# facebookresearch/AVID-CMA

Measured on AMD Instinct MI355X. Metric: clips/sec (video+audio fwd+bwd+NCE+Adam), higher is better.
Workload: dtype f32 (bf16x3 MFMA)

## Files before the change

avid-cma_amd/csrc/common.h:

```cpp
#pragma once
#include <hip/hip_runtime.h>
#include <stdint.h>
#include <stdio.h>
#include <string.h>

#include <mutex>

#include "../../include/avid_hip.h"

namespace avid {

typedef float floatx4 __attribute__((ext_vector_type(4)));
typedef float floatx16 __attribute__((ext_vector_type(16)));

void set_error(const char* fmt, ...);

inline int check_launch(const char* what) {
  hipError_t e = hipGetLastError();
  if (e != hipSuccess) {
    set_error("%s: %s", what, hipGetErrorString(e));
    return AVID_E_HIP;
  }
  return AVID_OK;
}

#define AVID_REQUIRE(cond, code, ...) \
  do {                                \
    if (!(cond)) {                    \
      avid::set_error(__VA_ARGS__);   \
      return (code);                  \
    }                                 \
  } while (0)

int device_cus();

inline int64_t ceil_div(int64_t a, int64_t b) { return (a + b - 1) / b; }

struct ScopedTimer {
  hipStream_t s;
  int slot;
  ScopedTimer(hipStream_t stream, const char* name, double flops, double bytes);
  ~ScopedTimer();
};

struct Stage {
  void* host = nullptr;
  size_t bytes = 0;
  hipEvent_t done = nullptr;
  bool used = false;
};
extern std::mutex g_stage_mu;
Stage* take_stage(size_t bytes);

int sim_gemm_nt(const float* A, const float* Bq, float* C, const float* Cin, int op, long long M, int N, int K,
                hipStream_t s);

bool stem_fwd_supported(const avid_conv_desc* d);
bool stem_wgrad_supported(const avid_conv_desc* d);
size_t stem_fwd_ws_bytes(const avid_conv_desc* d);
size_t stem_wgrad_ws_bytes(const avid_conv_desc* d);
int stem_fwd(const avid_conv_desc* d, const float* x, const float* w, float* y, float* stats, void* ws, hipStream_t s);
int stem_fwd_grid(const avid_conv_desc* d);
bool stem_fwd_is_split(const avid_conv_desc* d);
bool stem_fwd_is_presplit(const avid_conv_desc* d);
int stem_wgrad(const avid_conv_desc* d, const float* x, const float* dy, float* dw, void* ws, hipStream_t s);

bool wino_supported(const avid_conv_desc* d, int mode);
int wino_variant(const avid_conv_desc* d, int mode);
size_t wino_ws_bytes(const avid_conv_desc* d, int mode);
int wino_grid(const avid_conv_desc* d, int mode);
// ... 160 lines not shown
```

avid-cma_amd/csrc/common.hip:

```cpp
#include <stdarg.h>
#include <stdlib.h>

#include <map>
#include <string>
#include <vector>

#include <atomic>
#include "common.h"

namespace avid {
static thread_local char g_err[512] = "";

void set_error(const char* fmt, ...) {
  va_list ap;
  va_start(ap, fmt);
  vsnprintf(g_err, sizeof(g_err), fmt, ap);
  va_end(ap);
}

struct TimingRec {
  const char* name;
  double flops, bytes;
  hipEvent_t e0, e1;
};
static bool g_timing = false;
static std::vector<TimingRec> g_recs;
static std::vector<hipEvent_t> g_pool;

static hipEvent_t get_event() {
  if (!g_pool.empty()) {
    hipEvent_t e = g_pool.back();
    g_pool.pop_back();
    return e;
  }
  hipEvent_t e;
  (void)hipEventCreate(&e);
  return e;
}

ScopedTimer::ScopedTimer(hipStream_t stream, const char* name, double flops, double bytes) : s(stream), slot(-1) {
  if (!g_timing) return;
  TimingRec r{name, flops, bytes, get_event(), get_event()};
  (void)hipEventRecord(r.e0, s);
  slot = (int)g_recs.size();
  g_recs.push_back(r);
}
ScopedTimer::~ScopedTimer() {
  if (slot >= 0) (void)hipEventRecord(g_recs[slot].e1, s);
}

std::mutex g_stage_mu;
static std::vector<Stage> g_stages;

Stage* take_stage(size_t bytes) {
  for (auto& s : g_stages)
    if (s.bytes >= bytes && (!s.used || hipEventQuery(s.done) == hipSuccess)) return &s;
  Stage s;
  s.bytes = bytes < (1u << 20) ? (1u << 20) : bytes * 2;
  if (hipHostMalloc(&s.host, s.bytes, hipHostMallocDefault) != hipSuccess) return nullptr;
  if (hipEventCreateWithFlags(&s.done, hipEventDisableTiming) != hipSuccess) {
    (void)hipHostFree(s.host);
    return nullptr;
  }
  g_stages.push_back(s);
  return &g_stages.back();
}

static std::atomic<int> g_cu_budget{-1};

static int physical_cus() {
  static int cus[64] = {0};
// ... 93 lines not shown
```

avid-cma_amd/csrc/conv.hip:

```cpp
#include <math.h>
#include <stdlib.h>

#include <atomic>
#include <type_traits>

#include "common.h"

namespace avid {

typedef unsigned int uintx4 __attribute__((ext_vector_type(4)));

struct ConvArgs {
  const float* __restrict__ src;
  const float* __restrict__ wk;
  int w_row, w_nrec;
  const float* __restrict__ addend;
  const float* __restrict__ bias;
  float* __restrict__ dst;
  float* __restrict__ part;
  int B, Ts, Hs, Ws, Cs;
  int Td, Hd, Wd, Cd;
  int kt, kh, kw;
  int st, sh, sw;
  int pt, ph, pw;
  int M;
  int mode;
  int relu;
  int epi_op;
  int nsplit, ksteps_per_split;
  int mt2_begin, mt2_count;
  int part_row_begin;
  long long ssB, ssT, ssH, ssW, ssC;
  int ncls, cls_ptiles_total;
  int cls_begin[9];
  int cls_p0[8][3], cls_n[8][3];
  int cls_d0[8][3], cls_nd[8][3];
  unsigned mgW, mgH, mgT;
// ... 2437 lines not shown
  }
  reinterpret_cast<floatx4*>(dw)[i] = s;
}

__global__ __launch_bounds__(256) void dx_scatter_strided_kernel(const float* __restrict__ compact, const float* __restrict__ addend,
                                                                 float* __restrict__ dx, long long n4, int c4, int Ti, int Hi, int Wi,
                                                                 int To, int Ho, int Wo, int st, int sh, int sw) {
  for (long long i = (long long)blockIdx.x * 256 + threadIdx.x; i < n4; i += (long long)gridDim.x * 256) {
    const int c = (int)(i % c4);
    long long r = i / c4;
    const int w = (int)(r % Wi); r /= Wi;
    const int h = (int)(r % Hi); r /= Hi;
    const int t = (int)(r % Ti);
    const long long b = r / Ti;
    floatx4 v = {0.f, 0.f, 0.f, 0.f};
    if (t % st == 0 && h % sh == 0 && w % sw == 0)
      v = reinterpret_cast<const floatx4*>(compact)[((((b * To + t / st) * Ho + h / sh) * Wo + w / sw)) * c4 + c];
    if (addend) v += reinterpret_cast<const floatx4*>(addend)[i];
    reinterpret_cast<floatx4*>(dx)[i] = v;
  }
}

__global__ void weight_transpose_kernel(const float* __restrict__ w, float* __restrict__ wt, int Co, int ntaps, int Ci) {
  long long i = (long long)blockIdx.x * blockDim.x + threadIdx.x;
  long long n = (long long)Co * ntaps * Ci;
  if (i >= n) return;
  int co = (int)(i % Co);
  long long r = i / Co;
  int tap = (int)(r % ntaps);
  int ci = (int)(r / ntaps);
  wt[i] = w[((long long)co * ntaps + tap) * Ci + ci];
}

__device__ __forceinline__ void weight_transform_body(const avid_wt_desc& d, float (*tile)[33]) {
  if (d.mode >= 5) {
    const int N = d.mode == 5 ? d.Cout : d.Cin, C = d.mode == 5 ? d.Cin : d.Cout;
    const int c8 = C / 8, cpt = C / 32, ntn = N / 64;
    const long long items = (long long)N * d.ntaps * c8;
    char* out = reinterpret_cast<char*>(d.wt);
    for (long long i = (long long)blockIdx.x * 256 + threadIdx.x; i < items; i += (long long)gridDim.x * 256) {
      int n, tap, k8;
      float v[8];
      if (d.mode == 5) {
        k8 = (int)(i % c8);
        const long long r = i / c8;
        tap = (int)(r % d.ntaps);
        n = (int)(r / d.ntaps);
        const floatx4* src = reinterpret_cast<const floatx4*>(d.w + ((long long)n * d.ntaps + tap) * C + k8 * 8);
        const floatx4 a = src[0], b = src[1];
        v[0] = a[0]; v[1] = a[1]; v[2] = a[2]; v[3] = a[3]; v[4] = b[0]; v[5] = b[1]; v[6] = b[2]; v[7] = b[3];
      } else {
        n = (int)(i % N);
        const long long r = i / N;
        k8 = (int)(r % c8);
        tap = (int)(r / c8);
#pragma unroll
        for (int e = 0; e < 8; ++e) v[e] = d.w[((long long)(k8 * 8 + e) * d.ntaps + tap) * d.Cin + n];
      }
      pk_bf16x8 fh, fm, fl;
      pk_split8(floatx4{v[0], v[1], v[2], v[3]}, floatx4{v[4], v[5], v[6], v[7]}, fh, fm, fl);
      const int cb = k8 >> 2, st = (k8 >> 1) & 1, hh = k8 & 1;
      const long long chunk = ((long long)tap * cpt + cb) * ntn + (n >> 6);
      char* o = out + chunk * PK_BCH + ((((n >> 5) & 1) * 2 + st) * 3) * 1024 + (hh * 32 + (n & 31)) * 16;
      *reinterpret_cast<pk_bf16x8*>(o) = fh;
      *reinterpret_cast<pk_bf16x8*>(o + 1024) = fm;
      *reinterpret_cast<pk_bf16x8*>(o + 2048) = fl;
    }
    return;
  }
  if (d.mode != 0) {
    const bool fwd = d.mode & 1;
    wino_weight_elements(d.w, d.wt, fwd ? d.Cout : d.Cin, fwd ? d.Cin : d.Cout, d.Cin, !fwd,
                         (long long)blockIdx.x * 256 + threadIdx.x, (long long)gridDim.x * 256, d.mode <= 2 ? 2 : (W2_SPLIT ? 3 : 1));
    return;
  }
  const int tco = (d.Cout + 31) / 32, tci = (d.Cin + 31) / 32;
  const long long ntile = (long long)tco * tci * d.ntaps;
  const int tx = threadIdx.x & 31, ty = threadIdx.x >> 5;
  for (long long t = blockIdx.x; t < ntile; t += gridDim.x) {
    const int ci0 = (int)(t % tci) * 32;
    const long long r = t / tci;
    const int co0 = (int)(r % tco) * 32;
    const int tap = (int)(r / tco);
#pragma unroll
    for (int k = 0; k < 4; ++k) {
      const int co = co0 + ty + 8 * k, ci = ci0 + tx;
      tile[ty + 8 * k][tx] = (co < d.Cout && ci < d.Cin) ? d.w[((long long)co * d.ntaps + tap) * d.Cin + ci] : 0.f;
    }
    __syncthreads();
#pragma unroll
    for (int k = 0; k < 4; ++k) {
      const int ci = ci0 + ty + 8 * k, co = co0 + tx;
      if (ci < d.Cin && co < d.Cout) d.wt[((long long)ci * d.ntaps + tap) * d.Cout + co] = tile[tx][ty + 8 * k];
    }
    __syncthreads();
  }
}

__global__ __launch_bounds__(256) void weight_transpose_batched_kernel(const avid_wt_desc* __restrict__ descs) {
  __shared__ float tile[32][33];
  const avid_wt_desc d = descs[blockIdx.y];
  weight_transform_body(d, tile);
}

__global__ __launch_bounds__(256) void weight_transform_kernel(const avid_wt_desc d) {
  __shared__ float tile[32][33];
  weight_transform_body(d, tile);
}

static int validate(const avid_conv_desc* d) {
  AVID_REQUIRE(d != nullptr, AVID_E_BADARG, "conv: null descriptor");
  AVID_REQUIRE(d->B > 0 && d->Ti > 0 && d->Hi > 0 && d->Wi > 0 && d->Cin > 0 && d->Cout > 0, AVID_E_SHAPE,
               "conv: non-positive dims");
  AVID_REQUIRE(d->kt > 0 && d->kh > 0 && d->kw > 0 && d->kt < 256 && d->kh < 256 && d->kw < 256, AVID_E_SHAPE,
               "conv: bad kernel extent");
  AVID_REQUIRE(d->st > 0 && d->sh > 0 && d->sw > 0, AVID_E_SHAPE, "conv: bad stride");
  const int To = (d->Ti + 2 * d->pt - d->kt) / d->st + 1;
  const int Ho = (d->Hi + 2 * d->ph - d->kh) / d->sh + 1;
  const int Wo = (d->Wi + 2 * d->pw - d->kw) / d->sw + 1;
  AVID_REQUIRE(To == d->To && Ho == d->Ho && Wo == d->Wo, AVID_E_SHAPE,
               "conv: output extent (%d,%d,%d) does not match (%d,%d,%d)", d->To, d->Ho, d->Wo, To, Ho, Wo);
  AVID_REQUIRE(d->Cout % 64 == 0, AVID_E_UNSUPPORTED, "conv: Cout=%d must be a multiple of 64", d->Cout);
  const bool vec = (d->Cin % 32 == 0) && !d->x_channel_first;
  const int ntaps = d->kt * d->kh * d->kw;
  if (!vec) {
    AVID_REQUIRE(ntaps * d->Cin <= KTAB_MAX - 32, AVID_E_UNSUPPORTED,
                 "conv: gather path supports K <= %d (got %d)", KTAB_MAX - 32, ntaps * d->Cin);
  } else {
    AVID_REQUIRE(d->kt <= 8 && d->kh <= 8 && d->kw <= 8, AVID_E_UNSUPPORTED, "conv: vector path supports kernel extents <= 8");
    AVID_REQUIRE((long long)d->Cout * ntaps * d->Cin * 4 < (1ll << 31), AVID_E_UNSUPPORTED, "conv: weights >= 2 GiB");
  }
  const long long M = (long long)d->B * d->To * d->Ho * d->Wo;
  const long long Mi = (long long)d->B * d->Ti * d->Hi * d->Wi;
  AVID_REQUIRE(M < (1ll << 31) && Mi < (1ll << 31), AVID_E_UNSUPPORTED, "conv: more than 2^31 pixels");
  const long long pix_in = (long long)d->Ti * d->Hi * d->Wi, pix_out = (long long)d->To * d->Ho * d->Wo;
  const long long span_in = (128 / pix_out + 2) * pix_in * d->Cin * 4;
  const long long span_out = (128 / pix_in + 2) * pix_out * d->Cout * 4;
  AVID_REQUIRE(span_in < (1ll << 31) && span_out < (1ll << 31), AVID_E_UNSUPPORTED,
               "conv: one batch item is too large for 32-bit tile offsets");
  return AVID_OK;
// ... 959 lines not shown

static bool dgrad_compactable(const avid_conv_desc* d) {
  return d->kt == 1 && d->kh == 1 && d->kw == 1 && (d->st > 1 || d->sh > 1 || d->sw > 1) && d->pt == 0 && d->ph == 0 &&
         d->pw == 0 && !d->x_channel_first && d->Cin % 4 == 0;
}
static avid_conv_desc dgrad_compact_desc(const avid_conv_desc* d) {
  avid_conv_desc c = *d;
  c.Ti = d->To; c.Hi = d->Ho; c.Wi = d->Wo;
  c.st = c.sh = c.sw = 1;
  return c;
}
static size_t dgrad_compact_bytes(const avid_conv_desc* d) {
  return (sizeof(float) * (size_t)d->B * d->To * d->Ho * d->Wo * d->Cin + 255) / 256 * 256;
}

extern "C" size_t avid_conv_dgrad_workspace_bytes(const avid_conv_desc* d) {
  if (!d || validate(d)) return 0;
  if (dgrad_compactable(d)) {
    const avid_conv_desc c = dgrad_compact_desc(d);
    return dgrad_compact_bytes(d) + avid_conv_dgrad_workspace_bytes(&c);
  }
  const long long M = (long long)d->B * d->Ti * d->Hi * d->Wi;
  const int nk = trim_taps(d).d.kt * d->kh * d->kw * (d->Cout / BK);
  size_t fl = igemm_ws_floats(M, d->Cin, nk, 1);
  if (d->st > 1 || d->sh > 1 || d->sw > 1) {
    const size_t want = (size_t)8 * (size_t)M * d->Cin;
    if (want > fl) fl = want;
  }
  size_t need = dgrad_wt_bytes(d) + sizeof(float) * fl;
  if (wino_supported(d, 1) && wino_ws_bytes(d, 1) > need) need = wino_ws_bytes(d, 1);
  return need;
}

extern "C" int avid_weight_transpose_batched(int n, const avid_wt_desc* descs_dev, int64_t max_elems,
                                             avid_stream_t stream) {
  AVID_REQUIRE(n > 0 && descs_dev && max_elems > 0, AVID_E_BADARG, "weight_transpose_batched: bad argument");
  hipStream_t s = (hipStream_t)stream;
  ScopedTimer t(s, "weight_transpose_batched_kernel", 0.0, 0.0);
  long long gx = ceil_div(max_elems, 1024);
  if (gx > 256) gx = 256;
  hipLaunchKernelGGL(weight_transpose_batched_kernel, dim3((unsigned)gx, (unsigned)n), dim3(256), 0, s, descs_dev);
  return check_launch("weight_transpose_batched");
}

extern "C" int avid_weight_transform(const avid_wt_desc* desc, avid_stream_t stream) {
  AVID_REQUIRE(desc && desc->w && desc->wt && desc->Cout > 0 && desc->Cin > 0 && desc->ntaps > 0 && desc->mode >= 0 && desc->mode <= 6,
               AVID_E_BADARG, "weight_transform: bad descriptor");
  AVID_REQUIRE(desc->mode < 5 || (desc->mode == 5 ? desc->Cout % 64 == 0 && desc->Cin % 32 == 0 : desc->Cin % 64 == 0 && desc->Cout % 32 == 0),
               AVID_E_UNSUPPORTED, "weight_transform: mode %d needs 64 | rows and 32 | channels", desc->mode);
  hipStream_t s = (hipStream_t)stream;
  ScopedTimer t(s, "weight_transform_kernel", 0.0, 0.0);
  long long gx = ceil_div((long long)desc->Cout * desc->ntaps * desc->Cin, 1024);
  if (gx > 256) gx = 256;
  hipLaunchKernelGGL(weight_transform_kernel, dim3((unsigned)gx), dim3(256), 0, s, *desc);
  return check_launch("weight_transform");
}

extern "C" int avid_conv_dgrad_bn_rows(const avid_conv_desc* d) {
  if (!d || validate(d)) return 0;
  if (d->x_channel_first || d->Cin % 64 || d->Cout % 32 || d->st > 2 || d->sh > 2 || d->sw > 2) return 0;
  if (wino_supported(d, 1)) return wino_grid(d, 1);
  if (d->Cin > 1024 || (256 % (d->Cin / 4)) != 0) return 0;
  const long long M = (long long)d->B * d->Ti * d->Hi * d->Wi;
  if (d->st > 1 || d->sh > 1 || d->sw > 1) {
    if (M * d->Cin * 4 >= (1ll << 31)) return 0;
    const Trim tr = trim_taps(d);
    ConvArgs a{};
    fill_common(a, &tr.d);
    a.Td = d->Ti; a.Hd = d->Hi; a.Wd = d->Wi; a.Cd = d->Cin;
    const int BN = d->Cin % 128 == 0 && s2_wide() ? 128 : 64;
    a.Cs = d->Cout;
    a.M = (int)M;
    const StridedPlan pl = plan_strided(a, 128, BN, (size_t)8 * (size_t)M * d->Cin);
    return pl.grid + (pl.any_split ? (int)ceil_div(M, stats_rpb(M, d->Cin)) : 0);
  }
  const PkPlan pk = plan_pk(M, d->Cin, trim_taps(d).d.kt * d->kh * d->kw * (d->Cout / BK), 1);
  return pk.grid + (pk.f > 1 ? (int)ceil_div(M - pk.tail_row0, stats_rpb(M - pk.tail_row0, d->Cin)) : 0);
}

extern "C" int avid_conv_dgrad(const avid_conv_desc* d, const float* dy, const float* w, const float* wt_in,
                               const float* u, const float* addend, const int32_t* addend_stride, float* dx, const avid_bn_bwd_fuse* bn,
                               void* ws, size_t ws_bytes, avid_stream_t stream) {
  int rc = validate(d);
  if (rc) return rc;
// ... 545 lines not shown
```

avid-cma_amd/csrc/norm_pool.hip:

```cpp
#include <math.h>
#include <stdlib.h>

#include "common.h"

namespace avid {

struct BnPlan {
  int G;
  int rows_per_pass;
  int rows_per_block;
  int nblk;
};

static BnPlan bn_plan(int64_t M, int C) {
  BnPlan p;
  p.G = C / 4;
  p.rows_per_pass = 256 / p.G;
  int64_t rpb = ceil_div(M, 1024);
  if (rpb < 16) rpb = 16;
  rpb = ceil_div(rpb, p.rows_per_pass) * p.rows_per_pass;
  p.rows_per_block = (int)rpb;
  p.nblk = (int)ceil_div(M, rpb);
  return p;
}
// ... 602 lines not shown
    const int g = (int)(i % G);
    long long r = i / G;
    const int w = (int)(r % W);
    r /= W;
    const int h = (int)(r % H);
    const long long bt = r / H;
    floatx4 acc = {0, 0, 0, 0};
#pragma unroll
    for (int dh = 0; dh < 3; ++dh) {
      const int nh = h + 1 - dh;
      if (nh < 0 || (nh & 1)) continue;
      const int ho = nh >> 1;
      if (ho >= Ho) continue;
#pragma unroll
      for (int dw = 0; dw < 3; ++dw) {
        const int nw = w + 1 - dw;
        if (nw < 0 || (nw & 1)) continue;
        const int wo = nw >> 1;
        if (wo >= Wo) continue;
        const long long o = ((bt * Ho + ho) * Wo + wo) * (long long)G + g;
        const uchar4 a = reinterpret_cast<const uchar4*>(am)[o];
        const floatx4 d = reinterpret_cast<const floatx4*>(dy)[o];
        const int slot = dh * 3 + dw;
        acc.x += a.x == slot ? d.x : 0.f;
        acc.y += a.y == slot ? d.y : 0.f;
        acc.z += a.z == slot ? d.z : 0.f;
        acc.w += a.w == slot ? d.w : 0.f;
      }
    }
    reinterpret_cast<floatx4*>(dx)[i] = acc;
  }
}

__global__ __launch_bounds__(256) void bn_pool_fwd_kernel(const float* __restrict__ x, const float* __restrict__ scale,
                                                          const float* __restrict__ shift, float* __restrict__ y,
                                                          uint8_t* __restrict__ am, int BT, int H, int W, int Ho, int Wo,
                                                          int G) {
  const long long n = (long long)BT * Ho * Wo * G;
  const long long stride = (long long)gridDim.x * blockDim.x;
  for (long long i = (long long)blockIdx.x * blockDim.x + threadIdx.x; i < n; i += stride) {
    const int g = (int)(i % G);
    long long r = i / G;
    const int wo = (int)(r % Wo);
    r /= Wo;
    const int ho = (int)(r % Ho);
    const long long bt = r / Ho;
    const floatx4 sc = reinterpret_cast<const floatx4*>(scale)[g];
    const floatx4 sh = reinterpret_cast<const floatx4*>(shift)[g];
    floatx4 best = {-INFINITY, -INFINITY, -INFINITY, -INFINITY};
    int slot[4] = {0, 0, 0, 0};
    bool first = true;
#pragma unroll
    for (int dh = 0; dh < 3; ++dh) {
      const int h = ho * 2 - 1 + dh;
      if ((unsigned)h >= (unsigned)H) continue;
#pragma unroll
      for (int dw = 0; dw < 3; ++dw) {
        const int w = wo * 2 - 1 + dw;
        if ((unsigned)w >= (unsigned)W) continue;
        const floatx4 xv = *reinterpret_cast<const floatx4*>(x + (((bt * H + h) * W + w) * (long long)G + g) * 4);
#pragma unroll
        for (int j = 0; j < 4; ++j) {
          const float v = fmaxf(fmaf(xv[j], sc[j], sh[j]), 0.f);
          if (first || v > best[j] || v != v) {
            best[j] = v;
            slot[j] = dh * 3 + dw;
          }
        }
        first = false;
      }
    }
    reinterpret_cast<floatx4*>(y)[i] = best;
    reinterpret_cast<uchar4*>(am)[i] = make_uchar4((unsigned char)slot[0], (unsigned char)slot[1],
                                                   (unsigned char)slot[2], (unsigned char)slot[3]);
  }
}

__global__ __launch_bounds__(256) void bn_pool_fwd_eval_kernel(const float* __restrict__ x, const float* __restrict__ scale,
                                                               const float* __restrict__ shift, float* __restrict__ y,
                                                               int BT, int H, int W, int Ho, int Wo, int G) {
  const long long n = (long long)BT * Ho * Wo * G;
  const long long stride = (long long)gridDim.x * blockDim.x;
  for (long long i = (long long)blockIdx.x * blockDim.x + threadIdx.x; i < n; i += stride) {
    const int g = (int)(i % G);
    long long r = i / G;
    const int wo = (int)(r % Wo);
    r /= Wo;
    const int ho = (int)(r % Ho);
    const long long bt = r / Ho;
    const floatx4 sc = reinterpret_cast<const floatx4*>(scale)[g];
    const floatx4 sh = reinterpret_cast<const floatx4*>(shift)[g];
    floatx4 best = {-INFINITY, -INFINITY, -INFINITY, -INFINITY};
    bool first = true;
#pragma unroll
    for (int dh = 0; dh < 3; ++dh) {
      const int h = ho * 2 - 1 + dh;
      if ((unsigned)h >= (unsigned)H) continue;
#pragma unroll
      for (int dw = 0; dw < 3; ++dw) {
        const int w = wo * 2 - 1 + dw;
        if ((unsigned)w >= (unsigned)W) continue;
        const floatx4 xv = *reinterpret_cast<const floatx4*>(x + (((bt * H + h) * W + w) * (long long)G + g) * 4);
#pragma unroll
        for (int j = 0; j < 4; ++j) {
          const float v = fmaxf(fmaf(xv[j], sc[j], sh[j]), 0.f);
          if (first || v > best[j] || v != v) best[j] = v;
        }
        first = false;
      }
    }
    reinterpret_cast<floatx4*>(y)[i] = best;
  }
}

struct PoolCell {
  floatx4 d[2][2];
};
__device__ __forceinline__ PoolCell pool_cell_grad(const float* __restrict__ dy, const uint8_t* __restrict__ am,
                                                   long long bt, int a, int b, int g, int Ho, int Wo, int G) {
  uchar4 A[2][2];
  floatx4 D[2][2];
#pragma unroll
  for (int i = 0; i < 2; ++i)
#pragma unroll
    for (int j = 0; j < 2; ++j) {
      const bool ok = a + i < Ho && b + j < Wo;
      const long long o = ((bt * Ho + (ok ? a + i : 0)) * Wo + (ok ? b + j : 0)) * (long long)G + g;
      A[i][j] = reinterpret_cast<const uchar4*>(am)[o];
      D[i][j] = reinterpret_cast<const floatx4*>(dy)[o];
      if (!ok) A[i][j] = make_uchar4(255, 255, 255, 255);
    }
  PoolCell c;
  auto pick = [](uchar4 s, int slot, floatx4 d) {
    floatx4 r;
    r.x = s.x == slot ? d.x : 0.f; r.y = s.y == slot ? d.y : 0.f;
    r.z = s.z == slot ? d.z : 0.f; r.w = s.w == slot ? d.w : 0.f;
    return r;
  };
  c.d[0][0] = pick(A[0][0], 1 * 3 + 1, D[0][0]);
  c.d[0][1] = pick(A[0][0], 1 * 3 + 2, D[0][0]) + pick(A[0][1], 1 * 3 + 0, D[0][1]);
  c.d[1][0] = pick(A[0][0], 2 * 3 + 1, D[0][0]) + pick(A[1][0], 0 * 3 + 1, D[1][0]);
  c.d[1][1] = pick(A[0][0], 2 * 3 + 2, D[0][0]) + pick(A[0][1], 2 * 3 + 0, D[0][1]) + pick(A[1][0], 0 * 3 + 2, D[1][0]) +
              pick(A[1][1], 0 * 3 + 0, D[1][1]);
  return c;
}
// ... 258 lines not shown
                     running_mean, running_var, eps, n4, C / 4, relu);
  return check_launch("bn_fwd_eval");
}

extern "C" int avid_bn_eval_coeffs_batched(int n, const avid_bn_eval_item* items_dev, avid_stream_t stream) {
  static_assert(sizeof(BnEvalItem) == sizeof(avid_bn_eval_item), "BnEvalItem mirrors avid_bn_eval_item");
  AVID_REQUIRE(n > 0 && n <= 65535, AVID_E_SHAPE, "bn_eval_coeffs_batched: n=%d outside [1, 65535]", n);
  AVID_REQUIRE(items_dev, AVID_E_BADARG, "bn_eval_coeffs_batched: null table");
  ScopedTimer t((hipStream_t)stream, "bn_eval_coeff_batched_kernel", 0.0, 32.0 * n * 256);
  hipLaunchKernelGGL(bn_eval_coeff_batched_kernel, dim3(4, (unsigned)n), dim3(256), 0, (hipStream_t)stream,
                     reinterpret_cast<const BnEvalItem*>(items_dev));
  return check_launch("bn_eval_coeffs_batched");
}

extern "C" int avid_bn_apply_eval(int64_t M, int C, const float* x, const float* scale, const float* shift, int relu, float* y,
                                  avid_stream_t stream) {
  int rc = bn_check(M, C, "bn_apply_eval");
  if (rc) return rc;
  AVID_REQUIRE(x && scale && shift && y, AVID_E_BADARG, "bn_apply_eval: null pointer");
  const long long n4 = (long long)M * (C / 4);
  ScopedTimer t((hipStream_t)stream, "bn_apply_kernel", 0.0, 8.0 * M * C);
  hipLaunchKernelGGL(bn_apply_kernel, dim3(ew_grid(n4)), dim3(256), 0, (hipStream_t)stream, x, y, scale, shift, n4, C / 4, relu);
  return check_launch("bn_apply_eval");
}

extern "C" int avid_bn_relu_maxpool_fwd_eval(int B, int T, int H, int W, int C, const float* x, const float* scale,
                                             const float* shift, float* y, avid_stream_t stream) {
  const int64_t M = (int64_t)B * T * H * W;
  int rc = bn_check(M, C, "bn_relu_maxpool_fwd_eval");
  if (rc) return rc;
  AVID_REQUIRE(B > 0 && T > 0 && H > 0 && W > 0, AVID_E_SHAPE, "bn_relu_maxpool_fwd_eval: bad shape");
  AVID_REQUIRE(x && scale && shift && y, AVID_E_BADARG, "bn_relu_maxpool_fwd_eval: null pointer");
  const int Ho = (H + 2 - 3) / 2 + 1, Wo = (W + 2 - 3) / 2 + 1;
  const long long n = (long long)B * T * Ho * Wo * (C / 4);
  ScopedTimer t((hipStream_t)stream, "bn_pool_fwd_eval_kernel", 0.0, 4.0 * B * T * C * ((double)H * W + Ho * Wo));
  hipLaunchKernelGGL(bn_pool_fwd_eval_kernel, dim3(ew_grid(n)), dim3(256), 0, (hipStream_t)stream, x, scale, shift, y, B * T, H,
                     W, Ho, Wo, C / 4);
  return check_launch("bn_relu_maxpool_fwd_eval");
}

extern "C" int avid_bn_bwd(int64_t M, int C, const float* x, const float* dy, const float* gamma,
                           const float* save_mean, const float* save_invstd, const float* save_scale,
                           const float* save_shift, int relu, float* dx, float* dgamma, float* dbeta,
                           const float* partials, int nparts, int frozen, void* ws, size_t ws_bytes,
                           avid_stream_t stream) {
  int rc = bn_check(M, C, "bn_bwd");
  if (rc) return rc;
  AVID_REQUIRE(x && dy && gamma && save_mean && save_invstd && dx && dgamma && dbeta && ws, AVID_E_BADARG,
               "bn_bwd: null pointer");
  AVID_REQUIRE(!relu || (save_scale && save_shift), AVID_E_BADARG, "bn_bwd: relu needs the saved scale/shift");
  AVID_REQUIRE(ws_bytes >= avid_bn_workspace_bytes(M, C), AVID_E_BADARG, "bn_bwd: workspace too small");
  hipStream_t s = (hipStream_t)stream;
  BnPlan p = bn_plan(M, C);
  float* wsf = static_cast<float*>(ws);
  float* k1 = wsf + (size_t)p.nblk * 2 * C;
  float* k2 = k1 + C;
  const float* part = wsf;
  int nblk = p.nblk;
  if (partials && nparts > 0) {
    part = partials;
    nblk = nparts;
  } else {
    ScopedTimer t(s, "bn_bwd_partial_kernel", 0.0, 4.0 * M * C * 2);
    hipLaunchKernelGGL(bn_bwd_partial_kernel, dim3(p.nblk), dim3(256), 0, s, x, save_scale, save_shift, dy, save_mean,
                       save_invstd, wsf,
                       (long long)M, C, p.G, p.rows_per_pass, p.rows_per_block, relu);
  }
  if (bn_fused_ok(M, C)) {
    ScopedTimer t(s, "bn_bwd_fin_apply_kernel", 0.0, 4.0 * M * C * 3);
    hipLaunchKernelGGL(bn_bwd_fin_apply_kernel, dim3(bn_fused_grid(M, C)), dim3(256), 0, s, part, nblk, (long long)M, C, x,
// ... 17 lines not shown

extern "C" int avid_bn_relu_maxpool_fwd(int B, int T, int H, int W, int C, const float* x, const float* gamma,
                                        const float* beta, float* running_mean, float* running_var, float momentum,
                                        float eps, float* y, uint8_t* argmax, float* save_mean, float* save_invstd,
                                        float* save_scale, float* save_shift, int64_t* num_batches_tracked,
                                        const float* partials, int nparts, void* ws, size_t ws_bytes,
                                        avid_stream_t stream) {
  const int64_t M = (int64_t)B * T * H * W;
  int rc = bn_check(M, C, "bn_relu_maxpool_fwd");
  if (rc) return rc;
  AVID_REQUIRE(B > 0 && T > 0 && H > 0 && W > 0, AVID_E_SHAPE, "bn_relu_maxpool_fwd: bad shape");
  AVID_REQUIRE(x && gamma && beta && y && argmax && save_mean && save_invstd && save_scale && save_shift && ws,
               AVID_E_BADARG, "bn_relu_maxpool_fwd: null pointer");
  AVID_REQUIRE(ws_bytes >= avid_bn_workspace_bytes(M, C), AVID_E_BADARG, "bn_relu_maxpool_fwd: workspace too small");
  hipStream_t s = (hipStream_t)stream;
  BnPlan p = bn_plan(M, C);
  const float* part = static_cast<float*>(ws);
  int nblk = p.nblk;
  if (partials && nparts > 0) {
    part = partials;
    nblk = nparts;
  } else {
    ScopedTimer t(s, "bn_stats_partial_kernel", 0.0, 4.0 * M * C);
    hipLaunchKernelGGL(bn_stats_partial_kernel, dim3(p.nblk), dim3(256), 0, s, x, static_cast<float*>(ws), (long long)M,
                       C, p.G, p.rows_per_pass, p.rows_per_block);
  }
  {
    ScopedTimer t(s, "bn_finalize_kernel", 0.0, 8.0 * nblk * C);
    hipLaunchKernelGGL(bn_finalize_kernel, dim3((unsigned)ceil_div(C, FIN_CH)), dim3(1024), 0, s, part, nblk,
                       (long long)M, C, gamma, beta, running_mean, running_var, momentum, eps, save_mean, save_invstd,
                       save_scale, save_shift, reinterpret_cast<long long*>(num_batches_tracked));
  }
  const int Ho = (H + 2 - 3) / 2 + 1, Wo = (W + 2 - 3) / 2 + 1;
  const long long n = (long long)B * T * Ho * Wo * p.G;
  {
    ScopedTimer t(s, "bn_pool_fwd_kernel", 0.0, 4.0 * B * T * C * ((double)H * W + 1.25 * Ho * Wo));
    hipLaunchKernelGGL(bn_pool_fwd_kernel, dim3(ew_grid(n)), dim3(256), 0, s, x, save_scale, save_shift, y, argmax, B * T,
                       H, W, Ho, Wo, p.G);
  }
  return check_launch("bn_relu_maxpool_fwd");
}

extern "C" int avid_bn_relu_maxpool_bwd(int B, int T, int H, int W, int C, const float* x, const float* dy,
                                        const uint8_t* argmax, const float* gamma, const float* save_mean,
                                        const float* save_invstd, const float* save_scale, const float* save_shift,
                                        float* dx, float* dgamma, float* dbeta, void* ws, size_t ws_bytes,
                                        avid_stream_t stream) {
  const int64_t M = (int64_t)B * T * H * W;
  int rc = bn_check(M, C, "bn_relu_maxpool_bwd");
  if (rc) return rc;
  AVID_REQUIRE(x && dy && argmax && gamma && save_mean && save_invstd && save_scale && save_shift && dx && dgamma &&
                   dbeta && ws,
               AVID_E_BADARG, "bn_relu_maxpool_bwd: null pointer");
  AVID_REQUIRE(ws_bytes >= avid_bn_workspace_bytes(M, C), AVID_E_BADARG, "bn_relu_maxpool_bwd: workspace too small");
  hipStream_t s = (hipStream_t)stream;
  BnPlan p = bn_plan(M, C);
  const int Ho = (H + 2 - 3) / 2 + 1, Wo = (W + 2 - 3) / 2 + 1;
  float* part = static_cast<float*>(ws);
  float* k1 = part + (size_t)p.nblk * 2 * C;
  float* k2 = k1 + C;
  const long long cells = (long long)B * T * ((H + 1) / 2) * ((W + 1) / 2);
  long long cpb = ceil_div(cells, p.nblk);
  cpb = ceil_div(cpb, p.rows_per_pass) * p.rows_per_pass;
  const int nblk = (int)ceil_div(cells, cpb);
  {
    ScopedTimer t(s, "bn_pool_bwd_partial_kernel", 0.0, 4.0 * M * C * 1.3);
    hipLaunchKernelGGL(bn_pool_bwd_partial_kernel, dim3(nblk), dim3(256), 0, s, x, save_scale, save_shift, dy, argmax,
                       save_mean, save_invstd, part, cells, C, p.G, p.rows_per_pass, (int)cpb, H, W, Ho, Wo);
  }
  {
    ScopedTimer t(s, "bn_bwd_finalize_kernel", 0.0, 8.0 * nblk * C);
// ... 75 lines not shown
```

Measured before the change: 7016.

## Stage packed weight transform through LDS and band bn-relu-maxpool rows

The packed-bf16 weight transform (modes 5/6) now processes one 64x32 chunk per block. It loads the weights with coalesced vector reads into LDS and writes the hi/mid/lo fragments contiguously, replacing the old scattered per-thread gathers. The fused BN+ReLU+maxpool forward now gives each thread a vertical band of output rows. Each thread reuses the overlapping input row between adjacent pooling windows and prefetches the next rows, which cuts redundant loads and activation work at the cost of fewer threads. Timing instrumentation also gains byte counts, read through a host sync only when timing is on.

```diff
diff --git a/avid-cma_amd/csrc/common.h b/avid-cma_amd/csrc/common.h
--- a/avid-cma_amd/csrc/common.h
+++ b/avid-cma_amd/csrc/common.h
@@ -36,6 +36,7 @@
 
 inline int64_t ceil_div(int64_t a, int64_t b) { return (a + b - 1) / b; }
 
+bool timing_on();
 struct ScopedTimer {
   hipStream_t s;
   int slot;
diff --git a/avid-cma_amd/csrc/common.hip b/avid-cma_amd/csrc/common.hip
--- a/avid-cma_amd/csrc/common.hip
+++ b/avid-cma_amd/csrc/common.hip
@@ -37,6 +37,8 @@
   (void)hipEventCreate(&e);
   return e;
 }
+
+bool timing_on() { return g_timing; }
 
 ScopedTimer::ScopedTimer(hipStream_t stream, const char* name, double flops, double bytes) : s(stream), slot(-1) {
   if (!g_timing) return;
diff --git a/avid-cma_amd/csrc/conv.hip b/avid-cma_amd/csrc/conv.hip
--- a/avid-cma_amd/csrc/conv.hip
+++ b/avid-cma_amd/csrc/conv.hip
@@ -3,6 +3,7 @@
 
 #include <atomic>
 #include <type_traits>
+#include <vector>
 
 #include "common.h"
 
@@ -2506,39 +2507,55 @@
   wt[i] = w[((long long)co * ntaps + tap) * Ci + ci];
 }
 
-__device__ __forceinline__ void weight_transform_body(const avid_wt_desc& d, float (*tile)[33]) {
+constexpr int WT_SMEM = 64 * 36;
+__device__ __forceinline__ void weight_transform_body(const avid_wt_desc& d, float* smem) {
   if (d.mode >= 5) {
     const int N = d.mode == 5 ? d.Cout : d.Cin, C = d.mode == 5 ? d.Cin : d.Cout;
-    const int c8 = C / 8, cpt = C / 32, ntn = N / 64;
-    const long long items = (long long)N * d.ntaps * c8;
+    const int cpt = C / 32, ntn = N / 64;
+    const long long nchunk = (long long)d.ntaps * cpt * ntn;
     char* out = reinterpret_cast<char*>(d.wt);
-    for (long long i = (long long)blockIdx.x * 256 + threadIdx.x; i < items; i += (long long)gridDim.x * 256) {
-      int n, tap, k8;
-      float v[8];
+    const int t = threadIdx.x;
+    const int u = t & 63, q = t >> 6;
+    const int nhalf = q >> 1, st = q & 1, hh = u >> 5;
+    const int nrow = nhalf * 32 + (u & 31), k8l = st * 2 + hh;
+    for (long long chunk = blockIdx.x; chunk < nchunk; chunk += gridDim.x) {
+      const int nt = (int)(chunk % ntn);
+      const long long r = chunk / ntn;
+      const int cb = (int)(r % cpt), tap = (int)(r / cpt);
       if (d.mode == 5) {
-        k8 = (int)(i % c8);
-        const long long r = i / c8;
-        tap = (int)(r % d.ntaps);
-        n = (int)(r / d.ntaps);
-        const floatx4* src = reinterpret_cast<const floatx4*>(d.w + ((long long)n * d.ntaps + tap) * C + k8 * 8);
+        const int row = t >> 2, piece = t & 3;
+        const floatx4* src =
+            reinterpret_cast<const floatx4*>(d.w + ((long long)(nt * 64 + row) * d.ntaps + tap) * C + cb * 32 + piece * 8);
         const floatx4 a = src[0], b = src[1];
-        v[0] = a[0]; v[1] = a[1]; v[2] = a[2]; v[3] = a[3]; v[4] = b[0]; v[5] = b[1]; v[6] = b[2]; v[7] = b[3];
+        *reinterpret_cast<floatx4*>(smem + row * 36 + piece * 8) = a;
+        *reinterpret_cast<floatx4*>(smem + row * 36 + piece * 8 + 4) = b;
       } else {
-        n = (int)(i % N);
-        const long long r = i / N;
-        k8 = (int)(r % c8);
-        tap = (int)(r / c8);
-#pragma unroll
-        for (int e = 0; e < 8; ++e) v[e] = d.w[((long long)(k8 * 8 + e) * d.ntaps + tap) * d.Cin + n];
+        const int co = t >> 3, piece = t & 7;
+        const floatx4* src =
+            reinterpret_cast<const floatx4*>(d.w + ((long long)(cb * 32 + co) * d.ntaps + tap) * d.Cin + nt * 64 + piece * 8);
+        const floatx4 a = src[0], b = src[1];
+        *reinterpret_cast<floatx4*>(smem + co * 68 + piece * 8) = a;
+        *reinterpret_cast<floatx4*>(smem + co * 68 + piece * 8 + 4) = b;
+      }
+      __syncthreads();
+      floatx4 va, vb;
+      if (d.mode == 5) {
+        va = *reinterpret_cast<const floatx4*>(smem + nrow * 36 + k8l * 8);
+        vb = *reinterpret_cast<const floatx4*>(smem + nrow * 36 + k8l * 8 + 4);
+      } else {
+#pragma unroll
+        for (int e = 0; e < 4; ++e) {
+          va[e] = smem[(k8l * 8 + e) * 68 + nrow];
+          vb[e] = smem[(k8l * 8 + 4 + e) * 68 + nrow];
+        }
       }
       pk_bf16x8 fh, fm, fl;
-      pk_split8(floatx4{v[0], v[1], v[2], v[3]}, floatx4{v[4], v[5], v[6], v[7]}, fh, fm, fl);
-      const int cb = k8 >> 2, st = (k8 >> 1) & 1, hh = k8 & 1;
-      const long long chunk = ((long long)tap * cpt + cb) * ntn + (n >> 6);
-      char* o = out + chunk * PK_BCH + ((((n >> 5) & 1) * 2 + st) * 3) * 1024 + (hh * 32 + (n & 31)) * 16;
+      pk_split8(va, vb, fh, fm, fl);
+      char* o = out + chunk * PK_BCH + ((nhalf * 2 + st) * 3) * 1024 + u * 16;
       *reinterpret_cast<pk_bf16x8*>(o) = fh;
       *reinterpret_cast<pk_bf16x8*>(o + 1024) = fm;
       *reinterpret_cast<pk_bf16x8*>(o + 2048) = fl;
+      __syncthreads();
     }
     return;
   }
@@ -2548,6 +2565,7 @@
                          (long long)blockIdx.x * 256 + threadIdx.x, (long long)gridDim.x * 256, d.mode <= 2 ? 2 : (W2_SPLIT ? 3 : 1));
     return;
   }
+  float (*tile)[33] = reinterpret_cast<float (*)[33]>(smem);
   const int tco = (d.Cout + 31) / 32, tci = (d.Cin + 31) / 32;
   const long long ntile = (long long)tco * tci * d.ntaps;
   const int tx = threadIdx.x & 31, ty = threadIdx.x >> 5;
@@ -2572,14 +2590,14 @@
 }
 
 __global__ __launch_bounds__(256) void weight_transpose_batched_kernel(const avid_wt_desc* __restrict__ descs) {
-  __shared__ float tile[32][33];
+  __shared__ __attribute__((aligned(16))) float smem[WT_SMEM];
   const avid_wt_desc d = descs[blockIdx.y];
-  weight_transform_body(d, tile);
+  weight_transform_body(d, smem);
 }
 
 __global__ __launch_bounds__(256) void weight_transform_kernel(const avid_wt_desc d) {
-  __shared__ float tile[32][33];
-  weight_transform_body(d, tile);
+  __shared__ __attribute__((aligned(16))) float smem[WT_SMEM];
+  weight_transform_body(d, smem);
 }
 
 static int validate(const avid_conv_desc* d) {
@@ -3605,11 +3623,29 @@
   return need;
 }
 
+static double wt_desc_bytes(const avid_wt_desc& d) {
+  const double n = (double)d.Cout * d.ntaps * d.Cin;
+  if (d.mode == 0) return 8.0 * n;
+  if (d.mode >= 5) return 10.0 * n;
+  return (double)d.Cout * d.Cin * (36.0 + 96.0);
+}
+static double wt_table_bytes(int n, const avid_wt_desc* descs_dev, hipStream_t s) {
+  hipStreamCaptureStatus cap = hipStreamCaptureStatusNone;
+  if (hipStreamIsCapturing(s, &cap) != hipSuccess || cap != hipStreamCaptureStatusNone) return 0.0;
+  std::vector<avid_wt_desc> h((size_t)n);
+  if (hipMemcpyAsync(h.data(), descs_dev, sizeof(avid_wt_desc) * (size_t)n, hipMemcpyDeviceToHost, s) != hipSuccess ||
+      hipStreamSynchronize(s) != hipSuccess)
+    return 0.0;
+  double b = 0.0;
+  for (const avid_wt_desc& d : h) b += wt_desc_bytes(d);
+  return b;
+}
+
 extern "C" int avid_weight_transpose_batched(int n, const avid_wt_desc* descs_dev, int64_t max_elems,
                                              avid_stream_t stream) {
   AVID_REQUIRE(n > 0 && descs_dev && max_elems > 0, AVID_E_BADARG, "weight_transpose_batched: bad argument");
   hipStream_t s = (hipStream_t)stream;
-  ScopedTimer t(s, "weight_transpose_batched_kernel", 0.0, 0.0);
+  ScopedTimer t(s, "weight_transpose_batched_kernel", 0.0, timing_on() ? wt_table_bytes(n, descs_dev, s) : 0.0);
   long long gx = ceil_div(max_elems, 1024);
   if (gx > 256) gx = 256;
   hipLaunchKernelGGL(weight_transpose_batched_kernel, dim3((unsigned)gx, (unsigned)n), dim3(256), 0, s, descs_dev);
@@ -3622,7 +3658,7 @@
   AVID_REQUIRE(desc->mode < 5 || (desc->mode == 5 ? desc->Cout % 64 == 0 && desc->Cin % 32 == 0 : desc->Cin % 64 == 0 && desc->Cout % 32 == 0),
                AVID_E_UNSUPPORTED, "weight_transform: mode %d needs 64 | rows and 32 | channels", desc->mode);
   hipStream_t s = (hipStream_t)stream;
-  ScopedTimer t(s, "weight_transform_kernel", 0.0, 0.0);
+  ScopedTimer t(s, "weight_transform_kernel", 0.0, wt_desc_bytes(*desc));
   long long gx = ceil_div((long long)desc->Cout * desc->ntaps * desc->Cin, 1024);
   if (gx > 256) gx = 256;
   hipLaunchKernelGGL(weight_transform_kernel, dim3((unsigned)gx), dim3(256), 0, s, *desc);
diff --git a/avid-cma_amd/csrc/norm_pool.hip b/avid-cma_amd/csrc/norm_pool.hip
--- a/avid-cma_amd/csrc/norm_pool.hip
+++ b/avid-cma_amd/csrc/norm_pool.hip
@@ -658,85 +658,119 @@
   }
 }
 
+struct PoolRow {
+  floatx4 v;
+  int dw[4];
+};
+
+struct PoolFwdPlan {
+  int rows_per_band, nbh;
+  long long threads;
+};
+static PoolFwdPlan pool_fwd_plan(long long BT, int Ho, int Wo, int G) {
+  PoolFwdPlan p;
+  const long long per_level = BT * Wo * G;
+  long long nbh = (256ll * 28 * 64 + per_level - 1) / per_level;
+  if (nbh > Ho) nbh = Ho;
+  p.rows_per_band = (int)((Ho + nbh - 1) / nbh);
+  p.nbh = (Ho + p.rows_per_band - 1) / p.rows_per_band;
+  p.threads = per_level * p.nbh;
+  return p;
+}
+
+template <bool SLOTS>
+__device__ __forceinline__ void bn_pool_fwd_body(const float* __restrict__ x, const float* __restrict__ scale,
+                                                 const float* __restrict__ shift, float* __restrict__ y,
+                                                 uint8_t* __restrict__ am, long long n, int H, int W, int Ho, int Wo, int G,
+                                                 int rows_per_band, int nbh) {
+  const long long i = (long long)blockIdx.x * 256 + threadIdx.x;
+  if (i >= n) return;
+  const int g = (int)(i % G);
+  long long q = i / G;
+  const int wo = (int)(q % Wo);
+  q /= Wo;
+  const int hb = (int)(q % nbh);
+  const long long bt = q / nbh;
+  const int ho0 = hb * rows_per_band, ho1 = min(Ho, ho0 + rows_per_band);
+  const floatx4 sc = reinterpret_cast<const floatx4*>(scale)[g];
+  const floatx4 sh = reinterpret_cast<const floatx4*>(shift)[g];
+  const bool okl = wo > 0, okr = 2 * wo + 1 < W;
+  const long long cc = (long long)(2 * wo) * G + g, cl = okl ? cc - G : cc, cr = okr ? cc + G : cc;
+  const floatx4* frame = reinterpret_cast<const floatx4*>(x) + bt * H * (long long)W * G;
+  const floatx4 ninf = {-INFINITY, -INFINITY, -INFINITY, -INFINITY};
+  struct Raw { floatx4 e[3]; };
+  auto load = [&](int h) {
+    const floatx4* p = frame + (long long)h * W * G;
+    Raw r;
+    r.e[0] = p[cl]; r.e[1] = p[cc]; r.e[2] = p[cr];
+    return r;
+  };
+  auto act = [&](const floatx4& xv) {
+    floatx4 v;
+#pragma unroll
+    for (int j = 0; j < 4; ++j) v[j] = fmaxf(fmaf(xv[j], sc[j], sh[j]), 0.f);
+    return v;
+  };
+  auto reduce = [&](const Raw& r, bool ok) {
+    const floatx4 e0 = ok && okl ? act(r.e[0]) : ninf, e1 = ok ? act(r.e[1]) : ninf, e2 = ok && okr ? act(r.e[2]) : ninf;
+    PoolRow b;
+    b.v = e0;
+#pragma unroll
+    for (int j = 0; j < 4; ++j) {
+      b.dw[j] = 0;
+      if (e1[j] > b.v[j] || e1[j] != e1[j]) { b.v[j] = e1[j]; b.dw[j] = 1; }
+      if (e2[j] > b.v[j] || e2[j] != e2[j]) { b.v[j] = e2[j]; b.dw[j] = 2; }
+    }
+    return b;
+  };
+  PoolRow top;
+  if (ho0 > 0) {
+    top = reduce(load(2 * ho0 - 1), true);
+  } else {
+    top.v = ninf;
+#pragma unroll
+    for (int j = 0; j < 4; ++j) top.dw[j] = 0;
+  }
+  auto pool = [&](int ho, const Raw& r1, const Raw& r2) {
+    const PoolRow mid = reduce(r1, true), bot = reduce(r2, 2 * ho + 1 < H);
+    floatx4 best = top.v;
+    int slot[4];
+#pragma unroll
+    for (int j = 0; j < 4; ++j) {
+      slot[j] = top.dw[j];
+      if (mid.v[j] > best[j] || mid.v[j] != mid.v[j]) { best[j] = mid.v[j]; slot[j] = 3 + mid.dw[j]; }
+      if (bot.v[j] > best[j] || bot.v[j] != bot.v[j]) { best[j] = bot.v[j]; slot[j] = 6 + bot.dw[j]; }
+    }
+    const long long o = ((bt * Ho + ho) * Wo + wo) * (long long)G + g;
+    reinterpret_cast<floatx4*>(y)[o] = best;
+    if (SLOTS)
+      reinterpret_cast<uchar4*>(am)[o] = make_uchar4((unsigned char)slot[0], (unsigned char)slot[1],
+                                                     (unsigned char)slot[2], (unsigned char)slot[3]);
+    top = bot;
+  };
+  Raw a1 = load(2 * ho0), a2 = load(min(2 * ho0 + 1, H - 1));
+  int ho = ho0;
+  for (; ho + 1 < ho1; ++ho) {
+    const Raw b1 = load(2 * ho + 2), b2 = load(min(2 * ho + 3, H - 1));
+    pool(ho, a1, a2);
+    a1 = b1;
+    a2 = b2;
+  }
+  pool(ho, a1, a2);
+}
+
 __global__ __launch_bounds__(256) void bn_pool_fwd_kernel(const float* __restrict__ x, const float* __restrict__ scale,
                                                           const float* __restrict__ shift, float* __restrict__ y,
-                                                          uint8_t* __restrict__ am, int BT, int H, int W, int Ho, int Wo,
-                                                          int G) {
-  const long long n = (long long)BT * Ho * Wo * G;
-  const long long stride = (long long)gridDim.x * blockDim.x;
-  for (long long i = (long long)blockIdx.x * blockDim.x + threadIdx.x; i < n; i += stride) {
-    const int g = (int)(i % G);
-    long long r = i / G;
-    const int wo = (int)(r % Wo);
-    r /= Wo;
-    const int ho = (int)(r % Ho);
-    const long long bt = r / Ho;
-    const floatx4 sc = reinterpret_cast<const floatx4*>(scale)[g];
-    const floatx4 sh = reinterpret_cast<const floatx4*>(shift)[g];
-    floatx4 best = {-INFINITY, -INFINITY, -INFINITY, -INFINITY};
-    int slot[4] = {0, 0, 0, 0};
-    bool first = true;
-#pragma unroll
-    for (int dh = 0; dh < 3; ++dh) {
-      const int h = ho * 2 - 1 + dh;
-      if ((unsigned)h >= (unsigned)H) continue;
-#pragma unroll
-      for (int dw = 0; dw < 3; ++dw) {
-        const int w = wo * 2 - 1 + dw;
-        if ((unsigned)w >= (unsigned)W) continue;
-        const floatx4 xv = *reinterpret_cast<const floatx4*>(x + (((bt * H + h) * W + w) * (long long)G + g) * 4);
-#pragma unroll
-        for (int j = 0; j < 4; ++j) {
-          const float v = fmaxf(fmaf(xv[j], sc[j], sh[j]), 0.f);
-          if (first || v > best[j] || v != v) {
-            best[j] = v;
-            slot[j] = dh * 3 + dw;
-          }
-        }
-        first = false;
-      }
-    }
-    reinterpret_cast<floatx4*>(y)[i] = best;
-    reinterpret_cast<uchar4*>(am)[i] = make_uchar4((unsigned char)slot[0], (unsigned char)slot[1],
-                                                   (unsigned char)slot[2], (unsigned char)slot[3]);
-  }
+                                                          uint8_t* __restrict__ am, long long n, int H, int W, int Ho, int Wo,
+                                                          int G, int rows_per_band, int nbh) {
+  bn_pool_fwd_body<true>(x, scale, shift, y, am, n, H, W, Ho, Wo, G, rows_per_band, nbh);
 }
 
 __global__ __launch_bounds__(256) void bn_pool_fwd_eval_kernel(const float* __restrict__ x, const float* __restrict__ scale,
                                                                const float* __restrict__ shift, float* __restrict__ y,
-                                                               int BT, int H, int W, int Ho, int Wo, int G) {
-  const long long n = (long long)BT * Ho * Wo * G;
-  const long long stride = (long long)gridDim.x * blockDim.x;
-  for (long long i = (long long)blockIdx.x * blockDim.x + threadIdx.x; i < n; i += stride) {
-    const int g = (int)(i % G);
-    long long r = i / G;
-    const int wo = (int)(r % Wo);
-    r /= Wo;
-    const int ho = (int)(r % Ho);
-    const long long bt = r / Ho;
-    const floatx4 sc = reinterpret_cast<const floatx4*>(scale)[g];
-    const floatx4 sh = reinterpret_cast<const floatx4*>(shift)[g];
-    floatx4 best = {-INFINITY, -INFINITY, -INFINITY, -INFINITY};
-    bool first = true;
-#pragma unroll
-    for (int dh = 0; dh < 3; ++dh) {
-      const int h = ho * 2 - 1 + dh;
-      if ((unsigned)h >= (unsigned)H) continue;
-#pragma unroll
-      for (int dw = 0; dw < 3; ++dw) {
-        const int w = wo * 2 - 1 + dw;
-        if ((unsigned)w >= (unsigned)W) continue;
-        const floatx4 xv = *reinterpret_cast<const floatx4*>(x + (((bt * H + h) * W + w) * (long long)G + g) * 4);
-#pragma unroll
-        for (int j = 0; j < 4; ++j) {
-          const float v = fmaxf(fmaf(xv[j], sc[j], sh[j]), 0.f);
-          if (first || v > best[j] || v != v) best[j] = v;
-        }
-        first = false;
-      }
-    }
-    reinterpret_cast<floatx4*>(y)[i] = best;
-  }
+                                                               long long n, int H, int W, int Ho, int Wo, int G,
+                                                               int rows_per_band, int nbh) {
+  bn_pool_fwd_body<false>(x, scale, shift, y, nullptr, n, H, W, Ho, Wo, G, rows_per_band, nbh);
 }
 
 struct PoolCell {
@@ -1061,10 +1095,10 @@
   AVID_REQUIRE(B > 0 && T > 0 && H > 0 && W > 0, AVID_E_SHAPE, "bn_relu_maxpool_fwd_eval: bad shape");
   AVID_REQUIRE(x && scale && shift && y, AVID_E_BADARG, "bn_relu_maxpool_fwd_eval: null pointer");
   const int Ho = (H + 2 - 3) / 2 + 1, Wo = (W + 2 - 3) / 2 + 1;
-  const long long n = (long long)B * T * Ho * Wo * (C / 4);
   ScopedTimer t((hipStream_t)stream, "bn_pool_fwd_eval_kernel", 0.0, 4.0 * B * T * C * ((double)H * W + Ho * Wo));
-  hipLaunchKernelGGL(bn_pool_fwd_eval_kernel, dim3(ew_grid(n)), dim3(256), 0, (hipStream_t)stream, x, scale, shift, y, B * T, H,
-                     W, Ho, Wo, C / 4);
+  const PoolFwdPlan pp = pool_fwd_plan((long long)B * T, Ho, Wo, C / 4);
+  hipLaunchKernelGGL(bn_pool_fwd_eval_kernel, dim3((unsigned)ceil_div(pp.threads, 256)), dim3(256), 0, (hipStream_t)stream, x,
+                     scale, shift, y, pp.threads, H, W, Ho, Wo, C / 4, pp.rows_per_band, pp.nbh);
   return check_launch("bn_relu_maxpool_fwd_eval");
 }
 
@@ -1148,11 +1182,11 @@
                        save_scale, save_shift, reinterpret_cast<long long*>(num_batches_tracked));
   }
   const int Ho = (H + 2 - 3) / 2 + 1, Wo = (W + 2 - 3) / 2 + 1;
-  const long long n = (long long)B * T * Ho * Wo * p.G;
   {
     ScopedTimer t(s, "bn_pool_fwd_kernel", 0.0, 4.0 * B * T * C * ((double)H * W + 1.25 * Ho * Wo));
-    hipLaunchKernelGGL(bn_pool_fwd_kernel, dim3(ew_grid(n)), dim3(256), 0, s, x, save_scale, save_shift, y, argmax, B * T,
-                       H, W, Ho, Wo, p.G);
+    const PoolFwdPlan pp = pool_fwd_plan((long long)B * T, Ho, Wo, p.G);
+    hipLaunchKernelGGL(bn_pool_fwd_kernel, dim3((unsigned)ceil_div(pp.threads, 256)), dim3(256), 0, s, x, save_scale,
+                       save_shift, y, argmax, pp.threads, H, W, Ho, Wo, p.G, pp.rows_per_band, pp.nbh);
   }
   return check_launch("bn_relu_maxpool_fwd");
 }
```

Measured after the change: 7066, median of 6. Within noise of the previous version (+0.7%).
